# hiboyang/kueue_oss

Hardware: AMD Instinct MI355X
Metric: TAS placements/sec at 128k nodes (1/2/4/8 GPU); % HBM roofline (higher is better)
Workload: dtype int64; 1 GPU; C3: 131072 nodes, 1024 pending workloads per GPU per step from TASPodSetRequests (grouping + request compile + evaluation + TopologyAssignment values in the step; 50% BestFit required/preferred, 50% LeastFreeCapacity unconstrained; taints + nodeSelector); nodes=131072, batch_per_gpu=1024, parallelism=dp1 (replicated snapshot)

## Files before the change

include/kueue_tas.h:

```cpp
#ifndef KUEUE_TAS_H_
#define KUEUE_TAS_H_

#include <stddef.h>
#include <stdint.h>

#ifdef __cplusplus
extern "C" {
#endif

#define KUEUE_TAS_ABI_VERSION 5
#define KUEUE_TAS_MAX_LEVELS 16
#define KUEUE_TAS_MAX_COLS 32
#define KUEUE_TAS_MAX_SELECTORS 8
#define KUEUE_TAS_MAX_LAYERS 4

#define KUEUE_TAS_OK 0
#define KUEUE_TAS_EINVAL -1
#define KUEUE_TAS_ENOMEM -2
#define KUEUE_TAS_EDEVICE -3
#define KUEUE_TAS_ENOSNAPSHOT -4
#define KUEUE_TAS_EOVERFLOW -5
#define KUEUE_TAS_ELAYOUT -6
#define KUEUE_TAS_EHOSTMEM -7

// ... 94 lines not shown
  int32_t excl_affinity;
  int32_t excl_topology;
  int32_t ml_fit[KUEUE_TAS_MAX_LAYERS];
  int32_t ml_need[KUEUE_TAS_MAX_LAYERS];
  int32_t reserved[2];
} kueue_tas_eval_out;

typedef struct {
  int32_t list_cap;
  int32_t max_batch;
  int32_t device;
  int32_t flags;
} kueue_tas_config;
#define KUEUE_TAS_CFG_PACKED_ENTRIES 1
#define KUEUE_TAS_CFG_INLINE_STATS 2
#define KUEUE_TAS_CFG_NO_PAIR_FILL 4
#define KUEUE_TAS_CFG_SERIAL_ADMIT 8
#define KUEUE_TAS_CFG_SPLIT_STATS 16
#define KUEUE_TAS_CFG_FUSED_TOP 32
#define KUEUE_TAS_CFG_HOST_VALUES 64
#define KUEUE_TAS_CFG_NO_CATEGORY_FILL 128
#define KUEUE_TAS_CFG_CLASS_COLLIDE 256
#define KUEUE_TAS_CFG_LFC_IN_FILL 512

int kueue_tas_abi_version(void);
kueue_tas_ctx* kueue_tas_ctx_create(const kueue_tas_config* cfg);
void kueue_tas_ctx_destroy(kueue_tas_ctx* ctx);
const char* kueue_tas_last_error(kueue_tas_ctx* ctx);

int kueue_tas_snapshot_load(kueue_tas_ctx* ctx, const kueue_tas_snapshot_desc* desc);
int kueue_tas_snapshot_apply_deltas(kueue_tas_ctx* ctx, const kueue_tas_delta* deltas, size_t n,
                                    const uint32_t* usage_present_or_null);

int kueue_tas_snapshot_set_free(kueue_tas_ctx* ctx, const int32_t* leaves, size_t n, const int64_t* rows,
                                const uint32_t* free_present);

int kueue_tas_snapshot_set_leaf_attrs(kueue_tas_ctx* ctx, const int32_t* leaves, size_t n, const int32_t* profiles,
                                      const int32_t* labels);

int kueue_tas_snapshot_set_leaf_live(kueue_tas_ctx* ctx, const int32_t* leaves, size_t n, const int32_t* live);

#define KUEUE_TAS_DIGEST_CHUNK 2048
int kueue_tas_snapshot_digest(kueue_tas_ctx* ctx, uint64_t* words, size_t cap, size_t* len, uint64_t* chunks,
                              size_t chunk_cap, size_t* n_chunks);
int kueue_tas_snapshot_read_leaves(kueue_tas_ctx* ctx, const int32_t* leaves, size_t n, int64_t* free_rows,
                                   uint32_t* free_present, int64_t* usage_rows, uint32_t* usage_present,
// ... 170 lines not shown
```

include/kueue_tas_debug.h:

```cpp
#ifndef KUEUE_TAS_DEBUG_H_
#define KUEUE_TAS_DEBUG_H_

#include "kueue_tas.h"

#ifdef __cplusplus
extern "C" {
#endif

int kueue_tas_last_timings(kueue_tas_ctx* ctx, float* ms4);

#define KUEUE_TAS_NUM_STAGES 7
int kueue_tas_last_stage_times(kueue_tas_ctx* ctx, float* ms, int n);

int kueue_tas_last_eval_ticks(kueue_tas_ctx* ctx, int32_t* ticks, size_t n);

int kueue_tas_last_eval_profile(kueue_tas_ctx* ctx, int32_t* ticks, size_t n);
int64_t kueue_tas_last_fill_profile(kueue_tas_ctx* ctx, int32_t* out, size_t n);

int kueue_tas_last_host_times(kueue_tas_ctx* ctx, double* ms, int n);
int kueue_tas_last_host_trace(kueue_tas_ctx* ctx, double* ms, int n);
int64_t kueue_tas_merge_reruns(kueue_tas_ctx* ctx);
int kueue_tas_select_groups(kueue_tas_ctx* ctx, int64_t* last_groups, int64_t* scratch_reruns);
int kueue_tas_last_digest_ms(kueue_tas_ctx* ctx, float* ms2);

int kueue_tas_last_stats(kueue_tas_ctx* ctx, int64_t* stats4);
int64_t kueue_tas_last_alias_fills(kueue_tas_ctx* ctx);
#define KUEUE_TAS_PATH_STAGED 1u
#define KUEUE_TAS_PATH_STAGED_GLOBAL_TAINTS 2u
#define KUEUE_TAS_PATH_GENERIC4 4u
#define KUEUE_TAS_PATH_GENERIC8 8u
#define KUEUE_TAS_PATH_GENERIC16 16u
#define KUEUE_TAS_PATH_GENERIC32 32u
#define KUEUE_TAS_PATH_STAGED_GL 64u
#define KUEUE_TAS_PATH_GLOBAL_STATS 128u
#define KUEUE_TAS_PATH_EXCL 256u
#define KUEUE_TAS_PATH_EXCL_GLOBAL_TAINTS 512u
#define KUEUE_TAS_PATH_SELECTOR_EXT 1024u
#define KUEUE_TAS_PATH_RAGGED_ROLLUP 2048u
#define KUEUE_TAS_PATH_UNIFORM_ROLLUP 4096u
#define KUEUE_TAS_PATH_PAIR 8192u
#define KUEUE_TAS_PATH_ENTRY_TAGS 16384u
#define KUEUE_TAS_PATH_RAGGED_PAIR 32768u
#define KUEUE_TAS_PATH_CATEGORY 65536u
#define KUEUE_TAS_PATH_LFC_FILL 131072u
#define KUEUE_TAS_PATH_FUSED_TOP 262144u
uint32_t kueue_tas_last_fill_paths(kueue_tas_ctx* ctx);
uint64_t kueue_tas_eval_generation(kueue_tas_ctx* ctx);
int kueue_tas_set_stage_timing(kueue_tas_ctx* ctx, int32_t on);
int kueue_tas_snapshot_counters(kueue_tas_ctx* ctx, int64_t* loads, int64_t* splices);
int kueue_tas_device_bytes(kueue_tas_ctx* ctx, int64_t* total, int64_t* phase2);
int kueue_tas_snapshot_usage_mark(kueue_tas_ctx* ctx);
int kueue_tas_snapshot_usage_changes(kueue_tas_ctx* ctx, const kueue_tas_delta** changes, size_t* n);
int kueue_tas_snapshot_apply_deltas_mirrored(kueue_tas_ctx* ctx, const kueue_tas_delta* deltas, size_t n);

int kueue_tas_host_last_timings(kueue_tas_host* h, float* ms4, int64_t* counts3);
int kueue_tas_host_last_stage_times(kueue_tas_host* h, float* ms, int n);
int kueue_tas_host_last_device_host_times(kueue_tas_host* h, double* ms, int n);
int kueue_tas_host_last_eval_profile(kueue_tas_host* h, int32_t* ticks, size_t n);
int kueue_tas_host_last_eval_ticks(kueue_tas_host* h, int32_t* ticks, size_t n);
int kueue_tas_host_last_profile(kueue_tas_host* h, double* ms4);
int kueue_tas_host_last_host_detail(kueue_tas_host* h, double* ms, int n);
int kueue_tas_host_last_update_detail(kueue_tas_host* h, double* ms, int n);
int kueue_tas_host_set_stage_timing(kueue_tas_host* h, int32_t on);
int kueue_tas_host_stage_accum(kueue_tas_host* h, float* ms, int n, int64_t* runs, int64_t* fill_launches,
                               int32_t reset);
int kueue_tas_host_last_stats(kueue_tas_host* h, int64_t* stats8);
int kueue_tas_host_last_stats_ext(kueue_tas_host* h, int64_t* out, int32_t n);
int kueue_tas_host_last_counters(kueue_tas_host* h, size_t workload, int32_t* out, size_t cap);
// ... 13 lines not shown
```

kueue_oss_amd/abi.py:

```python
import ctypes as c

MAX_LEVELS = 16
MAX_COLS = 32
MAX_SELECTORS = 8
MAX_LAYERS = 4

F_REQUIRED = 1
F_UNCONSTRAINED = 2
F_LFC = 4
F_SIMULATE_EMPTY = 8
F_LEADER = 16
F_MULTILAYER = 32
F_AFFINITY = 64
F_DOMAIN = 128
F_SELECTOR_EXT = 256

ST_OK = 0
ST_NO_DOMAINS = 1
ST_NOT_FIT = 2
ST_MULTILAYER = 3
ST_INTERNAL = 4


class SnapshotDesc(c.Structure):
    _fields_ = [
        ("num_levels", c.c_int32),
        ("level_sizes", c.POINTER(c.c_int32)),
        ("child_offsets", c.POINTER(c.c_int32)),
        ("num_cols", c.c_int32),
        ("free_capacity", c.POINTER(c.c_int64)),
        ("tas_usage", c.POINTER(c.c_int64)),
        ("free_present", c.POINTER(c.c_uint32)),
        ("usage_present", c.POINTER(c.c_uint32)),
        ("lowest_is_hostname", c.c_int32),
        ("taint_profile", c.POINTER(c.c_int32)),
        ("num_label_cols", c.c_int32),
        ("label_values", c.POINTER(c.c_int32)),
        ("domain_id_rank", c.POINTER(c.c_int32)),
# ... 183 lines not shown
```

kueue_oss_amd/csrc/tas_device.hip:

```cpp
#include <hip/hip_runtime.h>

#include <algorithm>
#include <chrono>
#include <cstdio>
#include <cstring>
#include <string>
#include <mutex>
#include <unordered_map>
#include <vector>

#include "tas_internal.h"
#include "tas_pool.h"
#include "tas_kernels.hip"

using namespace ktas;

namespace {

constexpr int kEvalsPerFillBlock = kEvalsPerBlock;

bool simple_class(const DevEval& ev, int L) {
  bool simple = (ev.flags & KUEUE_TAS_F_LEADER) == 0 && ev.slice_level == L - 1 && ev.slice_size == 1;
  for (int l = 0; l < L && simple; l++) simple = ev.ssal[l] == 0 || ev.ssal[l] == 1;
  return simple;
// ... 149 lines not shown
  MagicSlot slot[256];
};
void compute_magic(uint64_t d, DevTerm* t, MagicCache& cache) {
  MagicSlot& c = cache.slot[(d * 0x9e3779b97f4a7c15ull) >> 56];
  if (c.d != d) {
    compute_magic_uncached(d, t);
    c.d = d;
    c.magic = t->magic;
    c.shift = t->shift;
    c.add = t->add;
    c.pow2 = t->pow2;
    return;
  }
  t->magic = c.magic;
  t->shift = c.shift;
  t->add = c.add;
  t->pow2 = c.pow2;
}

struct Knobs {
  int admit_grid_sweeps = 6;
  int admit_step_run = 2 * kAdmitWindow;
  int64_t phase2_budget = int64_t(4096) << 20;
  bool force_scratch_rerun = false;
  int64_t lcap_test_cap = 0;
  bool scratch_bounded = true;
  bool lfc_in_fill = false;
  bool emit_after_bf = false;
  int32_t exp_flags = 0;

  static Knobs from_env() {
    Knobs k;
    auto on = [](const char* name) {
      const char* e = getenv(name);
      return e && atoi(e) != 0;
    };
    if (const char* e = getenv("KTAS_ADMIT_PHASES")) k.admit_grid_sweeps = std::max(1, atoi(e));
    if (const char* e = getenv("KTAS_ADMIT_STEP_RUN")) k.admit_step_run = std::max(0, atoi(e));
    if (const char* e = getenv("KTAS_PHASE2_BUDGET")) k.phase2_budget = std::max<int64_t>(atoll(e), 1);
    k.force_scratch_rerun = getenv("KTAS_SCRATCH_TEST_RERUN") != nullptr;
    if (const char* e = getenv("KTAS_SCRATCH_TEST_CAP")) k.lcap_test_cap = std::max<int64_t>(atoll(e), 1);
    k.scratch_bounded = !on("KTAS_SCRATCH_FULL");
    k.lfc_in_fill = on("KTAS_LFC_IN_FILL");
    k.emit_after_bf = on("KTAS_EMIT_MAIN");
    if (const char* e = getenv("KTAS_EXP_FLAGS")) k.exp_flags = int32_t(atoi(e));
    return k;
  }
};

}

struct kueue_tas_ctx {
  int device = 0;
  hipStream_t stream = nullptr;
  hipStream_t stream2 = nullptr;
  hipStream_t stream3 = nullptr;
  hipEvent_t evs[2] = {};
  DevBuf<int8_t> d_fill_lim;
  std::vector<int32_t> cls_pos, cls_cur;
  hipEvent_t ev[8] = {};
  hipEvent_t evl[4] = {};
  std::string err;
  int list_cap = 1024;
  bool inline_stats = true;
  bool pair_fill = true;
  bool admit_window = true;
  Knobs knobs;
  bool fused_top = false;
  bool cat_fill = true;
  bool labels16 = false;
  int64_t n_loads = 0, n_splices = 0;
  bool stage_timing = true;
  int max_batch = 1024;
  int entry_cap = 512;
  bool loaded = false;
  DevSnap snap{};
  int maxD = 0;
  int rack_fanout = 0;
  std::vector<int32_t> h_level_sizes;
  DevBuf<int32_t> d_child_off, d_id_rank, d_taint_profile, d_labels;
  DevBuf<uint8_t> d_dead;
  std::vector<uint8_t> h_dead;
  int64_t n_dead = 0;
  DevBuf<int64_t> d_free, d_usage;
  DevBuf<uint32_t> d_free_present, d_usage_present;
  DevBuf<int32_t> d_counters;
  DevBuf<uint8_t> d_res;
  HostBuf<uint8_t> h_res;
  HostBuf<kueue_tas_eval_out> h_res2;
  kueue_tas_eval_out* res_out_h = nullptr;
  int32_t* res_stats_h = nullptr;
  DevBuf<uint64_t> d_scratch;
  DevBuf<kueue_tas_delta> d_deltas;
  DevBuf<uint8_t> d_setfree;
  DevBuf<uint8_t> d_fits;
  DevBuf<int32_t> d_parent;
  DevBuf<int2> d_wave_tab;
  DevBuf<int32_t> d_leaf_parent;
  DevBuf<char> d_names;
  DevBuf<int64_t> d_name_off;
  bool names_loaded = false;
  DevBuf<char> d_enc_bytes;
  DevBuf<int64_t> d_enc_stroff, d_enc_off;
  DevBuf<int32_t> d_enc_ids, d_enc_counts, d_enc_same;
  DevBuf<kueue_tas_level_enc> d_enc_out;
  DevBuf<int32_t> d_packed;
  DevBuf<LeafPartial> d_partials;
  DevBuf<int32_t> d_fill_stats;
  HostBuf<uint8_t> h_stage;
  DevBuf<uint8_t> d_stage;
  std::vector<int32_t> cls_rep, cls_sig, cls_of, sig_rep, cls_next, sig_next, cls_fastrep, cls_slot, cls_order;
  std::vector<int32_t> sig_base, base_rep, cls_packed, sig_ncls;
// ... 116 lines not shown
  } while (0)

extern "C" {

static double wall_ms() {
  return std::chrono::duration<double, std::milli>(std::chrono::steady_clock::now().time_since_epoch()).count();
}

int kueue_tas_abi_version(void) { return KUEUE_TAS_ABI_VERSION; }

kueue_tas_ctx* kueue_tas_ctx_create(const kueue_tas_config* cfg) {
  DevBufLink* chain = nullptr;
  g_devbuf_chain = &chain;
  auto* c = new kueue_tas_ctx();
  g_devbuf_chain = nullptr;
  c->dev_bufs = chain;
  c->knobs = Knobs::from_env();
  if (cfg) {
    c->device = cfg->device;
    c->inline_stats = (cfg->flags & KUEUE_TAS_CFG_INLINE_STATS) != 0 || (cfg->flags & KUEUE_TAS_CFG_SPLIT_STATS) == 0;
    c->pair_fill = (cfg->flags & KUEUE_TAS_CFG_NO_PAIR_FILL) == 0;
    c->admit_window = (cfg->flags & KUEUE_TAS_CFG_SERIAL_ADMIT) == 0;
    c->fused_top = (cfg->flags & KUEUE_TAS_CFG_FUSED_TOP) != 0;
    c->cat_fill = (cfg->flags & KUEUE_TAS_CFG_NO_CATEGORY_FILL) == 0;
    c->collide_test = (cfg->flags & KUEUE_TAS_CFG_CLASS_COLLIDE) != 0;
    if (cfg->flags & KUEUE_TAS_CFG_LFC_IN_FILL) c->knobs.lfc_in_fill = true;
    if (cfg->list_cap > 0) {
      int lc = 64;
      while (lc < cfg->list_cap && lc < 1024) lc <<= 1;
      c->list_cap = lc;
    }
    if (cfg->max_batch > 0) c->max_batch = cfg->max_batch;
  }
  int ndev = 0;
  if (hipGetDeviceCount(&ndev) != hipSuccess || ndev <= c->device) {
    c->err = "no HIP device available";
    delete c;
    return nullptr;
  }
  int prio_lo = 0, prio_hi = 0;
  if (hipSetDevice(c->device) != hipSuccess || hipDeviceGetStreamPriorityRange(&prio_lo, &prio_hi) != hipSuccess ||
      hipStreamCreateWithPriority(&c->stream, hipStreamNonBlocking, prio_hi) != hipSuccess ||
      hipStreamCreateWithPriority(&c->stream2, hipStreamNonBlocking, prio_hi) != hipSuccess ||
      hipStreamCreateWithPriority(&c->stream3, hipStreamNonBlocking, prio_lo) != hipSuccess) {
    delete c;
    return nullptr;
// ... 45 lines not shown
  c->d_enc_counts.release();
  c->d_enc_same.release();
  c->d_enc_out.release();
  c->d_packed.release();
  c->d_partials.release();
  c->d_fill_stats.release();
  c->h_stage.release();
  c->d_stage.release();
  c->d_overlay.release();
  c->d_rack_pos.release();
  c->d_tags.release();
  c->d_lfc_ch.release();
  c->d_lfc_cp.release();
  c->d_lfc_tot.release();
  c->d_lfc_ovs.release();
  c->d_lfc_ovtot.release();
  c->d_lfc_u8.release();
  c->d_lfc_jobs.release();
  c->d_lfc_items.release();
  c->d_prof.release();
  c->d_level_max.release();
  if (c->ent_host) (void)hipHostFree(c->ent_host);
  c->ent_host = c->ent_dev = nullptr;
  if (c->tag_host) (void)hipHostFree(c->tag_host);
  c->tag_host = c->tag_dev = nullptr;
  c->d_leaf_tags.release();
  for (auto& e : c->ev)
    if (e) (void)hipEventDestroy(e);
  for (auto& e : c->evl)
    if (e) (void)hipEventDestroy(e);
  for (auto& e : c->evs)
    if (e) (void)hipEventDestroy(e);
  if (c->ev_deltas) (void)hipEventDestroy(c->ev_deltas);
  for (auto& e : c->ev_digest)
    if (e) (void)hipEventDestroy(e);
  if (c->stream3) (void)hipStreamDestroy(c->stream3);
  if (c->stream2) (void)hipStreamDestroy(c->stream2);
  if (c->stream) (void)hipStreamDestroy(c->stream);
  delete c;
}

const char* kueue_tas_last_error(kueue_tas_ctx* c) { return c ? c->err.c_str() : "null ctx"; }

static int load_impl(kueue_tas_ctx* c, const kueue_tas_snapshot_desc* d, const kueue_tas_splice_desc* sp);

int kueue_tas_snapshot_load(kueue_tas_ctx* c, const kueue_tas_snapshot_desc* d) { return load_impl(c, d, nullptr); }
// ... 2239 lines not shown
      g_ov += ovf * SD;
      g_tag++;
      max_scr = std::max(max_scr, g_scr);
      max_ov = std::max(max_ov, g_ov);
      max_tag = std::max(max_tag, g_tag);
    }
    groups.push_back(nbf);
    HIPCHK(c, c->d_scratch.ensure(size_t(max_scr)));
    HIPCHK(c, c->d_overlay.ensure(size_t(max_ov)));
    const int ngroups = int(groups.size()) - 1;
    if (c->d_tags.n < size_t(max_tag) * size_t(SD) || c->tag_epoch + ngroups >= 0x7ffffff0) {
      HIPCHK(c, c->d_tags.ensure(size_t(max_tag) * size_t(SD)));
      HIPCHK(c, hipMemsetAsync(c->d_tags.p, 0, c->d_tags.n * 4, c->stream));
      c->tag_epoch = 0;
    }
  }
  c->tag_epoch++;
  const size_t nt = size_t(std::max(a.num_taints, 0));
  p.stats_len = n * nt + n * size_t(s.R) + 3 * n;
  p.res_off_stats = (n * sizeof(kueue_tas_eval_out) + 15) / 16 * 16;
  p.res_bytes = p.res_off_stats + p.stats_len * 4;
  HIPCHK(c, c->d_res.ensure(p.res_bytes));
  HIPCHK(c, c->h_res.ensure(p.res_bytes));
  HIPCHK(c, c->h_res2.ensure(n));
  c->res_out_h = reinterpret_cast<kueue_tas_eval_out*>(c->h_res.p);
  c->res_stats_h = reinterpret_cast<int32_t*>(c->h_res.p + p.res_off_stats);
  p.umask = 0;
  for (size_t i = 0; i < n; i++) p.umask |= hev[i].req_mask | hev[i].lead_mask;
  p.ucols = __builtin_popcount(p.umask);
  p.nstat_all = kStatFixed + int(nt) + s.R;
  p.lds_stats = s.N > 0 && p.nfchunks > 0 && p.ucols <= 8 && p.nstat_all <= kMaxFillStats;
  HIPCHK(c, c->d_lfc_jobs.ensure(n));
  HIPCHK(c, c->d_lfc_items.ensure(size_t(std::max(p.nfast, 1)) * size_t(std::max(nchunks, 1)) + 1));
  const size_t lfc_need = size_t(std::max(nslots * nchunks, 1));
  if (lfc_need > c->lfc_half) {
    c->lfc_half = lfc_need + lfc_need / 4;
    HIPCHK(c, c->d_lfc_ch.ensure(2 * c->lfc_half * kLfcBins));
    HIPCHK(c, c->d_lfc_ovs.ensure(2 * c->lfc_half));
    c->lfc_dirty[0] = c->lfc_dirty[1] = true;
  }
  p.lfc_cur = c->lfc_parity;
  HIPCHK(c, c->d_lfc_cp.ensure(size_t(std::max(nslots * nchunks, 1)) * kLfcBins));
  HIPCHK(c, c->d_lfc_tot.ensure(size_t(std::max(nslots, 1)) * kLfcBins));
  HIPCHK(c, c->d_lfc_ovtot.ensure(size_t(std::max(nslots, 1))));
  HIPCHK(c, c->d_lfc_u8.ensure(size_t(std::max(nslots, 1)) * size_t(std::max(nchunks, 1)) * kLfcChunk));
  p.nblk = (s.N + 255) / 256 * 4;
  HIPCHK(c, c->d_partials.ensure(size_t(std::max(p.nleafsel, 1)) * size_t(std::max(p.nblk, 1))));
  if (c->fused_top) {
// ... 165 lines not shown
  b.aff_vals = reinterpret_cast<const int32_t*>(ds + o.affv);
  b.n = int32_t(n);
  b.num_taints = int32_t(nt);
  b.num_profiles = c->num_profiles;
  b.nstat = 0;
  b.nstat_R = s.R;
  b.fill_stats = nullptr;
  b.stats_split = 0;
  b.fill_lim = nullptr;
  b.cls_member_off = nullptr;
  b.cls_members = nullptr;
  b.rack_fanout = 0;
  b.rack_pos = nullptr;
  b.ctr_sd = s.SD;
  b.counters = c->d_counters.p;
  b.overlay = c->d_overlay.p;
  b.tags = c->d_tags.p;
  b.tag_epoch = c->tag_epoch;
  b.taint_counts = d_stats;
  b.res_counts = d_stats + n * nt;
  b.sel_counts = d_stats + n * nt + n * size_t(s.R);
  b.aff_counts = b.sel_counts + n;
  b.dom_counts = b.aff_counts + n;
  b.out = d_out;
  b.entries = c->ent_dev + c->ent_used;
  b.entry_cap = c->entry_cap;
  b.sel_slots = reinterpret_cast<const SelSlot*>(ds + o.sel);
  b.slot_base = 0;
  b.scratch = c->d_scratch.p;
  b.list_cap = c->list_cap;
  b.nblk = p.nblk;
  b.partials = c->d_partials.p;
  b.partial_idx = reinterpret_cast<const int32_t*>(ds + o.pidx);
  b.rep_of = reinterpret_cast<const int32_t*>(ds + o.rep);
  b.lfc_slot = reinterpret_cast<const int32_t*>(ds + o.slot);
  b.lfc_rep = reinterpret_cast<const int32_t*>(ds + o.lrep);
  b.lfc_nslots = p.nslots;
  b.lfc_nchunks = p.nchunks;
  b.lfc_ch = c->d_lfc_ch.p + size_t(p.lfc_cur) * c->lfc_half * kLfcBins;
  b.lfc_u8 = c->d_lfc_u8.p;
  b.exp_flags = c->knobs.exp_flags;
  b.lfc_cp = c->d_lfc_cp.p;
  b.lfc_tot = c->d_lfc_tot.p;
  b.lfc_ovs = c->d_lfc_ovs.p + size_t(p.lfc_cur) * c->lfc_half;
  b.lfc_ovtot = c->d_lfc_ovtot.p;
  b.lfc_jobs = c->d_lfc_jobs.p;
  b.lfc_nitems = reinterpret_cast<int32_t*>(c->d_lfc_items.p);
// ... 210 lines not shown
  }
  return KUEUE_TAS_OK;
}

static int enqueue_rollup(kueue_tas_ctx* c, const ChunkArgs& a, const ChunkPlan& p, DevBatch& b) {
  const DevSnap& s = c->snap;
  const size_t n = a.n;
  const int nfill = p.nfill, nbf = p.nbf;
  uint8_t* ds = c->d_stage.p;
  const int upper = s.L - 2 - (b.rack_fanout ? 1 : 0);
  int top_parents = 0;
  for (int l = 0; l < upper; l++) top_parents += s.level_size[l];
  const bool fused_top = c->fused_top && nfill > 0 && upper >= 0 && s.level_size[upper] > 0 && top_parents <= 4096 &&
                         s.level_size[upper + 1] / s.level_size[upper] >= 8;
  if (fused_top) {
    c->fill_paths |= KUEUE_TAS_PATH_FUSED_TOP;
    b.level_max = nbf > 0 ? reinterpret_cast<int32_t*>(ds + p.o.top) : nullptr;
    const int per_block = 4 * kParentsPerWave;
    dim3 grid((s.level_size[upper] + per_block - 1) / per_block, unsigned(nfill));
    hipLaunchKernelGGL(rollup_top_kernel, grid, dim3(256), 0, c->stream, s, b, upper,
                       reinterpret_cast<int32_t*>(ds + p.o.top) + n * kMaxLevels);
    HIPCHK(c, hipGetLastError());
  }
  int tail_top = -1;
  if (!fused_top && nfill > 0)
    for (int l = upper; l >= 0 && tail_top < 0; l--)
      if (s.level_size[l] <= kTailParents) tail_top = l;
  for (int l = fused_top ? -1 : upper; l > tail_top; l--) {
    if (s.level_size[l] <= 0) continue;
    const int fanout = s.level_size[l + 1] / s.level_size[l];
    if (fanout >= 8) {
      const int per_block = 4 * kParentsPerWave;
      dim3 grid((s.level_size[l] + per_block - 1) / per_block, unsigned(nfill));
      hipLaunchKernelGGL(rollup_level_wave_kernel, grid, dim3(256), 0, c->stream, s, b, l);
    } else {
      dim3 grid((s.level_size[l] + 255) / 256, unsigned(nfill));
      hipLaunchKernelGGL(rollup_level_kernel, grid, dim3(256), 0, c->stream, s, b, l);
    }
    HIPCHK(c, hipGetLastError());
  }
  if (!fused_top && nfill > 0 && s.L >= 2 && (nbf > 0 || tail_top >= 0)) {
    b.level_max = nullptr;
    if (nbf > 0) {
      HIPCHK(c, c->d_level_max.ensure(size_t(nfill) * size_t(kMaxLevels)));
      b.level_max = c->d_level_max.p;
    }
// ... 67 lines not shown
    HIPCHK(c, hipStreamWaitEvent(c->stream2, c->ev[2], 0));
    if (c->stage_timing) HIPCHK(c, hipEventRecord(c->evl[0], c->stream2));
    if (!b.lfc_fill) {
      hipLaunchKernelGGL(lfc_hist_kernel, dim3(unsigned(nchunks), unsigned(nslots)), dim3(256), 0, c->stream2, s, b);
      HIPCHK(c, hipGetLastError());
    }
    hipLaunchKernelGGL(lfc_total_kernel, dim3(unsigned(nslots)), dim3(kLfcBins), 0, c->stream2, b);
    HIPCHK(c, hipGetLastError());
    if (stats_replicated(p, b)) HIPCHK(c, hipStreamWaitEvent(c->stream2, c->ev[4], 0));
    b.wave_lds = lfc_wave_lds(c);
    const SelSlot* sel = b.sel_slots;
    b.sel_slots = nullptr;
    hipLaunchKernelGGL(select_kernel, dim3(unsigned((nfast + waves - 1) / waves)), dim3(64 * waves),
                       size_t(waves) * size_t(b.wave_lds), c->stream2, s, b, dev_ints(c, p.o.fast), nfast);
    b.sel_slots = sel;
    HIPCHK(c, hipGetLastError());
    if (emit_main) {
      HIPCHK(c, hipEventRecord(c->evl[3], c->stream2));
    } else {
      hipLaunchKernelGGL(lfc_emit_kernel, dim3(unsigned(emit_grid)), dim3(256), 0, c->stream2, s, b);
      HIPCHK(c, hipGetLastError());
    }
    HIPCHK(c, hipEventRecord(c->evl[1], c->stream2));
    HIPCHK(c, hipMemcpyAsync(c->h_res2.p, c->d_res.p, n * sizeof(kueue_tas_eval_out), hipMemcpyDeviceToHost, c->stream2));
  }
  if (nfast && emit_main) {
    HIPCHK(c, hipStreamWaitEvent(c->stream, c->evl[3], 0));
    hipLaunchKernelGGL(lfc_emit_kernel, dim3(unsigned(emit_grid)), dim3(256), 0, c->stream, s, b);
    HIPCHK(c, hipGetLastError());
  }
  return KUEUE_TAS_OK;
}

static int enqueue_results_d2h(kueue_tas_ctx* c, const ChunkPlan& p, const DevBatch& b) {
  if (b.nstat > 0) HIPCHK(c, hipStreamWaitEvent(c->stream, c->evs[1], 0));
  if (c->stage_timing) HIPCHK(c, hipEventRecord(c->ev[7], c->stream));
  HIPCHK(c, hipMemcpyAsync(c->h_res.p, c->d_res.p, p.res_bytes, hipMemcpyDeviceToHost, c->stream));
  return KUEUE_TAS_OK;
}

static bool verify_merge(kueue_tas_ctx* c, const ChunkArgs& a, const ChunkPlan& p) {
  if (c->exact_merge) return true;
  const DevEval* hev = stage_evals(c, p);
  const ClassKeys keys(c, a, p);
  const std::vector<int32_t>& cls_rep = c->cls_rep;
  bool merge_ok = true;
  for (size_t t = 0; t < c->part_cls.size() && merge_ok; t++) {
    const PartClasses& pc = c->part_cls[t];
    for (size_t j = 0; j < pc.rep.size() && merge_ok; j++) {
      const int32_t r = cls_rep[size_t(c->part_map[c->part_base[t] + j])];
      if (r != pc.rep[j]) merge_ok = keys.same_sig(hev[pc.rep[j]], hev[r]) && keys.same_mask(hev[pc.rep[j]], hev[r]);
    }
  }
  for (size_t k = 0; k < cls_rep.size() && merge_ok; k++) {
    const int32_t g = c->sig_rep[size_t(c->cls_sig[k])];
    if (g != cls_rep[k]) merge_ok = keys.same_sig(hev[cls_rep[k]], hev[g]);
  }
  return merge_ok;
}

static int sync_and_check(kueue_tas_ctx* c, const ChunkPlan& p, bool merge_ok) {
  HIPCHK(c, hipStreamSynchronize(c->stream));
  if (p.nfast) {
    HIPCHK(c, hipStreamSynchronize(c->stream2));
    const int32_t* hf = stage_ints(c, p.o.fast);
    for (int k = 0; k < p.nfast; k++) c->res_out_h[hf[k]] = c->h_res2.p[hf[k]];
  }
  if (!merge_ok) {
    c->exact_merge = true;
    c->merge_reruns++;
    return ChunkRerun;
  }
  if (!c->scratch_full && c->knobs.scratch_bounded) {
    const int32_t* hb = stage_ints(c, p.o.bf);
    const SelSlot* hq = reinterpret_cast<const SelSlot*>(c->h_stage.p + p.o.sel);
    for (int k = 0; k < p.nbf; k++) {
      const kueue_tas_eval_out& o = c->res_out_h[hb[k]];
      if ((o.status == KUEUE_TAS_ST_INTERNAL && o.num_workers + o.num_leaders <= c->entry_cap && hq[k].lcap < p.full_lcap) ||
          c->knobs.force_scratch_rerun) {
        c->scratch_full = true;
        c->scratch_reruns++;
        return ChunkRerun;
      }
    }
  }
  return KUEUE_TAS_OK;
}

static int claim_entry_regions(kueue_tas_ctx* c, const ChunkArgs& a) {
  const size_t n = a.n;
// ... 464 lines not shown
```

kueue_oss_amd/csrc/tas_kernels.hip:

```cpp
#include <hip/hip_runtime.h>
#include <stdint.h>

#include <type_traits>

#include "tas_internal.h"

namespace ktas {

__device__ __forceinline__ int32_t w_add(int32_t a, int32_t b) { return int32_t(uint32_t(a) + uint32_t(b)); }
__device__ __forceinline__ int32_t w_sub(int32_t a, int32_t b) { return int32_t(uint32_t(a) - uint32_t(b)); }
__device__ __forceinline__ int32_t w_mul(int32_t a, int32_t b) { return int32_t(uint32_t(a) * uint32_t(b)); }
__device__ __forceinline__ int lane_id();
template <int M>
__device__ __forceinline__ uint32_t bfly(uint32_t v) {
  if constexpr (M == 1) return uint32_t(__builtin_amdgcn_update_dpp(0, int(v), 0xB1, 0xF, 0xF, false));
  else if constexpr (M == 2) return uint32_t(__builtin_amdgcn_update_dpp(0, int(v), 0x4E, 0xF, 0xF, false));
  else if constexpr (M == 4) return uint32_t(__builtin_amdgcn_update_dpp(0, int(v), 0x141, 0xF, 0xF, false));
  else if constexpr (M == 8) return uint32_t(__builtin_amdgcn_update_dpp(0, int(v), 0x140, 0xF, 0xF, false));
  else if constexpr (M == 16) {
    const auto r = __builtin_amdgcn_permlane16_swap(v, v, false, false);
    return uint32_t(r[0]) == v ? uint32_t(r[1]) : uint32_t(r[0]);
  } else {
    static_assert(M == 32, "butterfly steps are 1..32");
    const auto r = __builtin_amdgcn_permlane32_swap(v, v, false, false);
// ... 2169 lines not shown
    int4 v[U];
#pragma unroll
    for (int u = 0; u < U; u++) v[u] = ss4[min(q0 + u * 256 + int(threadIdx.x), nq - 1)];
#pragma unroll
    for (int u = 0; u < U; u++) {
      const int q = q0 + u * 256 + int(threadIdx.x);
      if (q < nq) {
        const int32_t e[4] = {v[u].x, v[u].y, v[u].z, v[u].w};
#pragma unroll
        for (int k = 0; k < 4; k++)
          if (4 * q + k < D) m = max(m, e[k]);
      }
    }
  }
  m = group_reduce(m, 64, OpMax());
  if (lane_id() == 0) red[threadIdx.x >> 6] = m;
  __syncthreads();
  if (threadIdx.x == 0) b.level_max[int64_t(row) * kMaxLevels + l] = max(max(red[0], red[1]), max(red[2], red[3]));
}

__device__ __forceinline__ int32_t load_l2_i32(const int32_t* p) {
  return __hip_atomic_load(p, __ATOMIC_RELAXED, __HIP_MEMORY_SCOPE_AGENT);
}
template <bool L2>
__device__ __forceinline__ void rollup_parent_wave(const DevSnap& s, int32_t* base, int64_t SSO, const DevEval& ev,
                                                   bool leaderReq, int level, int p, int32_t* cmax) {
  const int cl = level + 1;
  const int32_t inner = ev.ssal[cl];
  const bool hasInner = inner != 0;
  const int64_t SD = s.SD;
  const int coff = s.level_off[cl];
  const int lane = lane_id();
  const int cb = s.child_off[s.child_base[level] + p];
  const int ce = s.child_off[s.child_base[level] + p + 1];
  auto ld = [&](int64_t o) { return L2 ? load_l2_i32(base + o) : base[o]; };
  int32_t cap = 0, slc = 0, minD = 0x7fffffff, minSD = 0x7fffffff, lead = 0, mx = INT32_MIN;
  int has = 0;
  for (int c = cb + lane; c < ce; c += kWave) {
    const int g = coff + c;
    int32_t cs = ld(g);
    const int32_t css = ld(SSO + g);
    int32_t csw = cs, csswl = css, cls = 0;
    if (leaderReq) {
      csw = ld(2 * SD + g);
      csswl = ld(3 * SD + g);
      cls = ld(4 * SD + g);
    }
    mx = max(mx, css);
    if (hasInner) {
      cs = w_mul(go_div32(cs, inner), inner);
      csw = w_mul(go_div32(csw, inner), inner);
    }
    cap = w_add(cap, cs);
    slc = w_add(slc, css);
    if (!leaderReq || cls > 0) {
      has = 1;
      minD = min(w_sub(cs, csw), minD);
      minSD = min(w_sub(css, csswl), minSD);
    }
    lead = max(cls, lead);
  }
#pragma unroll
  for (int m = 1; m <= 32; m <<= 1) {
    cap = w_add(cap, xor_lane(cap, m));
    slc = w_add(slc, xor_lane(slc, m));
    minD = min(minD, xor_lane(minD, m));
    minSD = min(minSD, xor_lane(minSD, m));
    lead = max(lead, xor_lane(lead, m));
    has |= xor_lane(has, m);
    mx = max(mx, xor_lane(mx, m));
  }
  *cmax = max(*cmax, mx);
  if (lane == 0) {
    const int32_t state = cap;
    const int32_t swl = has ? w_sub(cap, minD) : 0;
    int32_t sswl = has ? w_sub(slc, minSD) : 0;
    if (level == ev.slice_level) {
      slc = go_div32(state, ev.slice_size);
      sswl = go_div32(swl, ev.slice_size);
    }
    const int g = s.level_off[level] + p;
    base[g] = state;
    if (SSO) base[SD + g] = slc;
    if (leaderReq) {
      base[2 * SD + g] = swl;
      base[3 * SD + g] = sswl;
      base[4 * SD + g] = lead;
    }
  }
}

__global__ __launch_bounds__(256) void rollup_top_kernel(DevSnap s, DevBatch b, int level, int32_t* arrivals) {
  __shared__ int32_t red[4];
  __shared__ int32_t last;
  const int row = blockIdx.y;
  const int eid = b.fill_ids[row];
  const DevEval& ev = b.evals[eid];
  const bool leaderReq = (ev.flags & KUEUE_TAS_F_LEADER) != 0;
  int32_t* base = ctr_base(b, row);
  const int64_t SSO = ss_off(b, row, s.SD);
  const int wv = threadIdx.x >> 6;
  int32_t cmax = INT32_MIN;
  const int p0 = (blockIdx.x * 4 + wv) * kParentsPerWave;
  for (int j = 0; j < kParentsPerWave; j++) {
    const int p = p0 + j;
    if (p < s.level_size[level]) rollup_parent_wave<false>(s, base, SSO, ev, leaderReq, level, p, &cmax);
  }
  if (lane_id() == 0) red[wv] = cmax;
  __syncthreads();
  if (threadIdx.x == 0) {
    const int32_t m = max(max(red[0], red[1]), max(red[2], red[3]));
    if (level + 1 < s.L - 1 && b.level_max) atomicMax(&b.level_max[int64_t(row) * kMaxLevels + level + 1], m);
// ... 41 lines not shown
    const int32_t* ss = base + SSO + s.level_off[l];
    int32_t m = INT32_MIN;
    if (l <= top) {
      for (int i = threadIdx.x; i < s.level_size[l]; i += 256) m = max(m, load_l2_i32(ss + i));
    } else {
      const int D = s.level_size[l];
      const int nq = (D + 3) / 4;
      const int4* ss4 = reinterpret_cast<const int4*>(ss);
      constexpr int U = 4;
      for (int q0 = 0; q0 < nq; q0 += U * 256) {
        int4 v[U];
#pragma unroll
        for (int u = 0; u < U; u++) v[u] = ss4[min(q0 + u * 256 + int(threadIdx.x), nq - 1)];
#pragma unroll
        for (int u = 0; u < U; u++) {
          const int q = q0 + u * 256 + int(threadIdx.x);
          const int32_t e[4] = {v[u].x, v[u].y, v[u].z, v[u].w};
#pragma unroll
          for (int k = 0; k < 4; k++)
            if (q < nq && 4 * q + k < D) m = max(m, e[k]);
        }
      }
    }
    m = group_reduce(m, 64, OpMax());
    if (lane_id() == 0) red[wv] = m;
    __syncthreads();
    if (threadIdx.x == 0) b.level_max[int64_t(row) * kMaxLevels + l] = max(max(red[0], red[1]), max(red[2], red[3]));
    __syncthreads();
  }
}

__global__ __launch_bounds__(kFillThreads) void leaf_partials_kernel(DevSnap s, DevBatch b, const int32_t* ids,
                                                                    int nids) {
  const int e0 = blockIdx.y * kEvalsPerBlock;
  const int ne = min(kEvalsPerBlock, nids - e0);
  const int leaf = blockIdx.x * kFillThreads + threadIdx.x;
  const bool valid = leaf < s.N;
  const int gleaf = s.level_off[s.L - 1] + leaf;
  const int lane = lane_id();
  const int64_t SD = s.SD;
  for (int e = 0; e < ne; e++) {
    const int eid = uni(ids[e0 + e]);
    const DevEval& ev = b.evals[eid];
    const uint32_t flags = uint32_t(uni(int32_t(ev.flags)));
    const bool leader = (flags & KUEUE_TAS_F_LEADER) != 0;
    const bool lfc = (flags & KUEUE_TAS_F_LFC) != 0;
// ... 4067 lines not shown
```

kueue_oss_amd/native.py:

```python
from __future__ import annotations

import ctypes
import json
import os
import subprocess

_PKG = os.path.dirname(os.path.abspath(__file__))
_CSRC = os.path.join(_PKG, "csrc")
_BUILD = os.path.join(_PKG, "_build")
_LIB = None


class NativeLibraryMissing(RuntimeError):
    """libkueue_tas.so could not be loaded or no HIP device is usable."""


def library_path() -> str:
    return os.path.join(_BUILD, "libkueue_tas.so")


def build_native(jobs: int = 4) -> str:
    subprocess.run(["make", "-s", f"-j{jobs}", "-C", _CSRC], check=True)
    return library_path()

# ... 207 lines not shown


def resource_quantity_string(name: str, value: int, lib=None) -> str:
    lib = lib if lib is not None else load_library()
    buf = ctypes.create_string_buffer(64)
    n = ctypes.c_size_t()
    if lib.kueue_tas_resource_quantity_string(name.encode(), value, buf, 64, ctypes.byref(n)):
        raise RuntimeError("kueue_tas_resource_quantity_string failed")
    return buf.value.decode()


def _take(lib, p) -> dict:
    s = ctypes.cast(p, ctypes.c_char_p).value.decode()
    lib.kueue_tas_free(p)
    return json.loads(s)


class TASFlavorSnapshot:

    def __init__(self, snapshot: dict, list_cap: int = 0, max_batch: int = 0, device: int = 0, lib=None,
                 packed_entries: bool = False, inline_stats: bool = False,
                 pair_fill: bool = True, serial_admit: bool = False, split_stats: bool = False,
                 fused_top: bool = False, host_values: bool = False, category_fill: bool = True,
                 class_collide: bool = False, lfc_in_fill: bool = False):
        self._lib = lib if lib is not None else load_library()
        cfg = KueueTasConfig(list_cap, max_batch, device, (1 if packed_entries else 0) | (2 if inline_stats else 0)
                              | (0 if pair_fill else 4) | (8 if serial_admit else 0) | (16 if split_stats else 0)
                              | (32 if fused_top else 0) | (64 if host_values else 0)
                              | (0 if category_fill else 128) | (256 if class_collide else 0)
                              | (512 if lfc_in_fill else 0))
        doc = {k: v for k, v in snapshot.items() if k != "podSets"}
        h = self._lib.kueue_tas_host_create(json.dumps(doc).encode(), ctypes.byref(cfg))
        if not h:
            raise NativeLibraryMissing("kueue_tas_host_create returned NULL")
        err = self._lib.kueue_tas_host_last_error(h).decode()
        if err:
            self._lib.kueue_tas_host_destroy(h)
            raise NativeLibraryMissing(err)
        self._h = h

    def close(self):
        if getattr(self, "_h", None):
            self._lib.kueue_tas_host_destroy(self._h)
            self._h = None

    def __del__(self):
        try:
            self.close()
        except Exception:
            pass

    def _err(self):
        return self._lib.kueue_tas_host_last_error(self._h).decode()
# ... 452 lines not shown
```

Baseline: 3.692 million placements/s.

## Write eval results to mapped host memory; add optional LDS block rollup kernel

```diff
diff --git a/include/kueue_tas.h b/include/kueue_tas.h
--- a/include/kueue_tas.h
+++ b/include/kueue_tas.h
@@ -140,6 +140,8 @@
 #define KUEUE_TAS_CFG_NO_CATEGORY_FILL 128
 #define KUEUE_TAS_CFG_CLASS_COLLIDE 256
 #define KUEUE_TAS_CFG_LFC_IN_FILL 512
+#define KUEUE_TAS_CFG_BLOCK_ROLLUP 1024
+#define KUEUE_TAS_CFG_COPY_RESULTS 2048
 
 int kueue_tas_abi_version(void);
 kueue_tas_ctx* kueue_tas_ctx_create(const kueue_tas_config* cfg);
diff --git a/include/kueue_tas_debug.h b/include/kueue_tas_debug.h
--- a/include/kueue_tas_debug.h
+++ b/include/kueue_tas_debug.h
@@ -44,6 +44,7 @@
 #define KUEUE_TAS_PATH_CATEGORY 65536u
 #define KUEUE_TAS_PATH_LFC_FILL 131072u
 #define KUEUE_TAS_PATH_FUSED_TOP 262144u
+#define KUEUE_TAS_PATH_BLOCK_ROLLUP 524288u
 uint32_t kueue_tas_last_fill_paths(kueue_tas_ctx* ctx);
 uint64_t kueue_tas_eval_generation(kueue_tas_ctx* ctx);
 int kueue_tas_set_stage_timing(kueue_tas_ctx* ctx, int32_t on);
diff --git a/kueue_oss_amd/abi.py b/kueue_oss_amd/abi.py
--- a/kueue_oss_amd/abi.py
+++ b/kueue_oss_amd/abi.py
@@ -14,6 +14,11 @@
 F_AFFINITY = 64
 F_DOMAIN = 128
 F_SELECTOR_EXT = 256
+
+CFG_BLOCK_ROLLUP = 1024
+CFG_COPY_RESULTS = 2048
+
+PATH_BLOCK_ROLLUP = 1 << 19
 
 ST_OK = 0
 ST_NO_DOMAINS = 1
diff --git a/kueue_oss_amd/csrc/tas_device.hip b/kueue_oss_amd/csrc/tas_device.hip
--- a/kueue_oss_amd/csrc/tas_device.hip
+++ b/kueue_oss_amd/csrc/tas_device.hip
@@ -195,6 +195,8 @@
   int admit_grid_sweeps = 6;
   int admit_step_run = 2 * kAdmitWindow;
   int64_t phase2_budget = int64_t(4096) << 20;
+  bool block_rollup = false;
+  int64_t rollup_lds_budget = 12288;
   bool force_scratch_rerun = false;
   int64_t lcap_test_cap = 0;
   bool scratch_bounded = true;
@@ -211,11 +213,13 @@
     if (const char* e = getenv("KTAS_ADMIT_PHASES")) k.admit_grid_sweeps = std::max(1, atoi(e));
     if (const char* e = getenv("KTAS_ADMIT_STEP_RUN")) k.admit_step_run = std::max(0, atoi(e));
     if (const char* e = getenv("KTAS_PHASE2_BUDGET")) k.phase2_budget = std::max<int64_t>(atoll(e), 1);
+    if (const char* e = getenv("KTAS_ROLLUP_LDS_BUDGET")) k.rollup_lds_budget = std::max<int64_t>(atoll(e), 0);
     k.force_scratch_rerun = getenv("KTAS_SCRATCH_TEST_RERUN") != nullptr;
     if (const char* e = getenv("KTAS_SCRATCH_TEST_CAP")) k.lcap_test_cap = std::max<int64_t>(atoll(e), 1);
     k.scratch_bounded = !on("KTAS_SCRATCH_FULL");
     k.lfc_in_fill = on("KTAS_LFC_IN_FILL");
     k.emit_after_bf = on("KTAS_EMIT_MAIN");
+    k.block_rollup = on("KTAS_BLOCK_ROLLUP");
     if (const char* e = getenv("KTAS_EXP_FLAGS")) k.exp_flags = int32_t(atoi(e));
     return k;
   }
@@ -240,6 +244,7 @@
   bool admit_window = true;
   Knobs knobs;
   bool fused_top = false;
+  bool mapped_results = true;
   bool cat_fill = true;
   bool labels16 = false;
   int64_t n_loads = 0, n_splices = 0;
@@ -261,6 +266,9 @@
   DevBuf<uint8_t> d_res;
   HostBuf<uint8_t> h_res;
   HostBuf<kueue_tas_eval_out> h_res2;
+  kueue_tas_eval_out* res_map_host = nullptr;
+  kueue_tas_eval_out* res_map_dev = nullptr;
+  size_t res_map_cap = 0;
   kueue_tas_eval_out* res_out_h = nullptr;
   int32_t* res_stats_h = nullptr;
   DevBuf<uint64_t> d_scratch;
@@ -423,6 +431,8 @@
     c->pair_fill = (cfg->flags & KUEUE_TAS_CFG_NO_PAIR_FILL) == 0;
     c->admit_window = (cfg->flags & KUEUE_TAS_CFG_SERIAL_ADMIT) == 0;
     c->fused_top = (cfg->flags & KUEUE_TAS_CFG_FUSED_TOP) != 0;
+    if (cfg->flags & KUEUE_TAS_CFG_BLOCK_ROLLUP) c->knobs.block_rollup = true;
+    c->mapped_results = (cfg->flags & KUEUE_TAS_CFG_COPY_RESULTS) == 0;
     c->cat_fill = (cfg->flags & KUEUE_TAS_CFG_NO_CATEGORY_FILL) == 0;
     c->collide_test = (cfg->flags & KUEUE_TAS_CFG_CLASS_COLLIDE) != 0;
     if (cfg->flags & KUEUE_TAS_CFG_LFC_IN_FILL) c->knobs.lfc_in_fill = true;
@@ -514,6 +524,8 @@
   c->d_level_max.release();
   if (c->ent_host) (void)hipHostFree(c->ent_host);
   c->ent_host = c->ent_dev = nullptr;
+  if (c->res_map_host) (void)hipHostFree(c->res_map_host);
+  c->res_map_host = c->res_map_dev = nullptr;
   if (c->tag_host) (void)hipHostFree(c->tag_host);
   c->tag_host = c->tag_dev = nullptr;
   c->d_leaf_tags.release();
@@ -2799,8 +2811,21 @@
   p.res_bytes = p.res_off_stats + p.stats_len * 4;
   HIPCHK(c, c->d_res.ensure(p.res_bytes));
   HIPCHK(c, c->h_res.ensure(p.res_bytes));
-  HIPCHK(c, c->h_res2.ensure(n));
-  c->res_out_h = reinterpret_cast<kueue_tas_eval_out*>(c->h_res.p);
+  if (c->mapped_results) {
+    if (n > c->res_map_cap) {
+      const size_t cap = std::max<size_t>(n, 2 * c->res_map_cap);
+      kueue_tas_eval_out* q = nullptr;
+      HIPCHK(c, hipHostMalloc(&q, cap * sizeof(kueue_tas_eval_out), hipHostMallocMapped | hipHostMallocCoherent));
+      if (c->res_map_host) (void)hipHostFree(c->res_map_host);
+      c->res_map_host = q;
+      c->res_map_cap = cap;
+      HIPCHK(c, hipHostGetDevicePointer(reinterpret_cast<void**>(&c->res_map_dev), q, 0));
+    }
+    c->res_out_h = c->res_map_host;
+  } else {
+    HIPCHK(c, c->h_res2.ensure(n));
+    c->res_out_h = reinterpret_cast<kueue_tas_eval_out*>(c->h_res.p);
+  }
   c->res_stats_h = reinterpret_cast<int32_t*>(c->h_res.p + p.res_off_stats);
   p.umask = 0;
   for (size_t i = 0; i < n; i++) p.umask |= hev[i].req_mask | hev[i].lead_mask;
@@ -3012,7 +3037,7 @@
   b.sel_counts = d_stats + n * nt + n * size_t(s.R);
   b.aff_counts = b.sel_counts + n;
   b.dom_counts = b.aff_counts + n;
-  b.out = d_out;
+  b.out = c->mapped_results ? c->res_map_dev : d_out;
   b.entries = c->ent_dev + c->ent_used;
   b.entry_cap = c->entry_cap;
   b.sel_slots = reinterpret_cast<const SelSlot*>(ds + o.sel);
@@ -3269,6 +3294,25 @@
                        reinterpret_cast<int32_t*>(ds + p.o.top) + n * kMaxLevels);
     HIPCHK(c, hipGetLastError());
   }
+  if (c->knobs.block_rollup && !fused_top && nfill > 0 && upper >= 0 && s.level_size[upper + 1] > 0) {
+    int64_t fields = 1;
+    for (int k = 0; k < nfill; k++) fields = std::max<int64_t>(fields, c->ctr_row_off[size_t(k) + 1] - c->ctr_row_off[size_t(k)]);
+    const int64_t mirror = fields * s.level_off[upper + 2];
+    if (fields * s.level_size[upper + 1] <= c->knobs.rollup_lds_budget && mirror <= kBlockRollupLarge) {
+      c->fill_paths |= KUEUE_TAS_PATH_BLOCK_ROLLUP;
+      b.level_max = nullptr;
+      if (nbf > 0) {
+        HIPCHK(c, c->d_level_max.ensure(size_t(nfill) * size_t(kMaxLevels)));
+        b.level_max = c->d_level_max.p;
+      }
+      if (mirror <= kBlockRollupSmall)
+        hipLaunchKernelGGL(rollup_block_kernel<kBlockRollupSmall>, dim3(unsigned(nfill)), dim3(256), 0, c->stream, s, b, upper);
+      else
+        hipLaunchKernelGGL(rollup_block_kernel<kBlockRollupLarge>, dim3(unsigned(nfill)), dim3(256), 0, c->stream, s, b, upper);
+      HIPCHK(c, hipGetLastError());
+      return KUEUE_TAS_OK;
+    }
+  }
   int tail_top = -1;
   if (!fused_top && nfill > 0)
     for (int l = upper; l >= 0 && tail_top < 0; l--)
@@ -3382,7 +3426,8 @@
       HIPCHK(c, hipGetLastError());
     }
     HIPCHK(c, hipEventRecord(c->evl[1], c->stream2));
-    HIPCHK(c, hipMemcpyAsync(c->h_res2.p, c->d_res.p, n * sizeof(kueue_tas_eval_out), hipMemcpyDeviceToHost, c->stream2));
+    if (!c->mapped_results)
+      HIPCHK(c, hipMemcpyAsync(c->h_res2.p, c->d_res.p, n * sizeof(kueue_tas_eval_out), hipMemcpyDeviceToHost, c->stream2));
   }
   if (nfast && emit_main) {
     HIPCHK(c, hipStreamWaitEvent(c->stream, c->evl[3], 0));
@@ -3393,6 +3438,14 @@
 }
 
 static int enqueue_results_d2h(kueue_tas_ctx* c, const ChunkPlan& p, const DevBatch& b) {
+  if (c->mapped_results) {
+    if (c->stage_timing) HIPCHK(c, hipEventRecord(c->ev[7], c->stream));
+    if (b.nstat == 0) HIPCHK(c, hipStreamWaitEvent(c->stream3, stats_replicated(p, b) ? c->ev[4] : c->ev[2], 0));
+    if (p.stats_len)
+      HIPCHK(c, hipMemcpyAsync(c->h_res.p + p.res_off_stats, c->d_res.p + p.res_off_stats, p.stats_len * 4,
+                               hipMemcpyDeviceToHost, c->stream3));
+    return KUEUE_TAS_OK;
+  }
   if (b.nstat > 0) HIPCHK(c, hipStreamWaitEvent(c->stream, c->evs[1], 0));
   if (c->stage_timing) HIPCHK(c, hipEventRecord(c->ev[7], c->stream));
   HIPCHK(c, hipMemcpyAsync(c->h_res.p, c->d_res.p, p.res_bytes, hipMemcpyDeviceToHost, c->stream));
@@ -3423,9 +3476,12 @@
   HIPCHK(c, hipStreamSynchronize(c->stream));
   if (p.nfast) {
     HIPCHK(c, hipStreamSynchronize(c->stream2));
-    const int32_t* hf = stage_ints(c, p.o.fast);
-    for (int k = 0; k < p.nfast; k++) c->res_out_h[hf[k]] = c->h_res2.p[hf[k]];
-  }
+    if (!c->mapped_results) {
+      const int32_t* hf = stage_ints(c, p.o.fast);
+      for (int k = 0; k < p.nfast; k++) c->res_out_h[hf[k]] = c->h_res2.p[hf[k]];
+    }
+  }
+  if (c->mapped_results) HIPCHK(c, hipStreamSynchronize(c->stream3));
   if (!merge_ok) {
     c->exact_merge = true;
     c->merge_reruns++;
diff --git a/kueue_oss_amd/csrc/tas_kernels.hip b/kueue_oss_amd/csrc/tas_kernels.hip
--- a/kueue_oss_amd/csrc/tas_kernels.hip
+++ b/kueue_oss_amd/csrc/tas_kernels.hip
@@ -2215,29 +2215,37 @@
 __device__ __forceinline__ int32_t load_l2_i32(const int32_t* p) {
   return __hip_atomic_load(p, __ATOMIC_RELAXED, __HIP_MEMORY_SCOPE_AGENT);
 }
-template <bool L2>
-__device__ __forceinline__ void rollup_parent_wave(const DevSnap& s, int32_t* base, int64_t SSO, const DevEval& ev,
-                                                   bool leaderReq, int level, int p, int32_t* cmax) {
+#if defined(__HIP_DEVICE_COMPILE__)
+typedef __attribute__((address_space(3))) int32_t lds_i32;
+#else
+typedef int32_t lds_i32;
+#endif
+template <bool L2, bool MIR = false>
+__device__ __forceinline__ void rollup_parent_range(const DevSnap& s, int32_t* base, int64_t SSO, bool leaderReq, int level,
+                                                    int32_t inner, bool at_slice, int32_t slice_size, int p, int cb, int ce,
+                                                    int32_t* cmax, lds_i32* mirror = nullptr, int MSD = 0) {
   const int cl = level + 1;
-  const int32_t inner = ev.ssal[cl];
   const bool hasInner = inner != 0;
   const int64_t SD = s.SD;
   const int coff = s.level_off[cl];
   const int lane = lane_id();
-  const int cb = s.child_off[s.child_base[level] + p];
-  const int ce = s.child_off[s.child_base[level] + p + 1];
-  auto ld = [&](int64_t o) { return L2 ? load_l2_i32(base + o) : base[o]; };
+  const int MSS = SSO ? MSD : 0;
+  auto ld = [&](int f, int g) {
+    if (MIR) return int32_t(mirror[(f == 1 ? MSS : f * MSD) + g]);
+    const int64_t o = (f == 1 ? SSO : f * SD) + g;
+    return L2 ? load_l2_i32(base + o) : base[o];
+  };
   int32_t cap = 0, slc = 0, minD = 0x7fffffff, minSD = 0x7fffffff, lead = 0, mx = INT32_MIN;
   int has = 0;
   for (int c = cb + lane; c < ce; c += kWave) {
     const int g = coff + c;
-    int32_t cs = ld(g);
-    const int32_t css = ld(SSO + g);
+    int32_t cs = ld(0, g);
+    const int32_t css = ld(1, g);
     int32_t csw = cs, csswl = css, cls = 0;
     if (leaderReq) {
-      csw = ld(2 * SD + g);
-      csswl = ld(3 * SD + g);
-      cls = ld(4 * SD + g);
+      csw = ld(2, g);
+      csswl = ld(3, g);
+      cls = ld(4, g);
     }
     mx = max(mx, css);
     if (hasInner) {
@@ -2268,9 +2276,9 @@
     const int32_t state = cap;
     const int32_t swl = has ? w_sub(cap, minD) : 0;
     int32_t sswl = has ? w_sub(slc, minSD) : 0;
-    if (level == ev.slice_level) {
-      slc = go_div32(state, ev.slice_size);
-      sswl = go_div32(swl, ev.slice_size);
+    if (at_slice) {
+      slc = go_div32(state, slice_size);
+      sswl = go_div32(swl, slice_size);
     }
     const int g = s.level_off[level] + p;
     base[g] = state;
@@ -2280,7 +2288,24 @@
       base[3 * SD + g] = sswl;
       base[4 * SD + g] = lead;
     }
-  }
+    if (MIR) {
+      mirror[g] = state;
+      if (SSO) mirror[MSD + g] = slc;
+      if (leaderReq) {
+        mirror[2 * MSD + g] = swl;
+        mirror[3 * MSD + g] = sswl;
+        mirror[4 * MSD + g] = lead;
+      }
+    }
+  }
+}
+template <bool L2>
+__device__ __forceinline__ void rollup_parent_wave(const DevSnap& s, int32_t* base, int64_t SSO, const DevEval& ev,
+                                                   bool leaderReq, int level, int p, int32_t* cmax) {
+  const int cb = s.child_off[s.child_base[level] + p];
+  const int ce = s.child_off[s.child_base[level] + p + 1];
+  rollup_parent_range<L2>(s, base, SSO, leaderReq, level, ev.ssal[level + 1], level == ev.slice_level, ev.slice_size, p, cb,
+                          ce, cmax);
 }
 
 __global__ __launch_bounds__(256) void rollup_top_kernel(DevSnap s, DevBatch b, int level, int32_t* arrivals) {
@@ -2368,6 +2393,72 @@
         }
       }
     }
+    m = group_reduce(m, 64, OpMax());
+    if (lane_id() == 0) red[wv] = m;
+    __syncthreads();
+    if (threadIdx.x == 0) b.level_max[int64_t(row) * kMaxLevels + l] = max(max(red[0], red[1]), max(red[2], red[3]));
+    __syncthreads();
+  }
+}
+
+constexpr int kBlockRollupSmall = 5120;
+constexpr int kBlockRollupLarge = 15360;
+template <int CAP>
+__global__ __launch_bounds__(256) void rollup_block_kernel(DevSnap s, DevBatch b, int upper) {
+  __shared__ int32_t mirror[CAP];
+  __shared__ int32_t red[4];
+  const int row = blockIdx.x;
+  const DevEval& ev = b.evals[b.fill_ids[row]];
+  const bool leaderReq = (ev.flags & KUEUE_TAS_F_LEADER) != 0;
+  int32_t* base = ctr_base(b, row);
+  const int64_t SD = s.SD;
+  const int64_t SSO = ss_off(b, row, SD);
+  const int nf = leaderReq ? 5 : SSO ? 2 : 1;
+  const int cl = upper + 1;
+  const int MSD = s.level_off[cl + 1];
+  const int wv = threadIdx.x >> 6;
+  {
+    const int coff = s.level_off[cl];
+    const int nq = (s.level_size[cl] + 3) / 4;
+    const int total = nf * nq;
+    constexpr int U = 4;
+    for (int q0 = 0; q0 < total; q0 += U * 256) {
+      int4 v[U];
+#pragma unroll
+      for (int u = 0; u < U; u++) {
+        const int i = min(q0 + u * 256 + int(threadIdx.x), total - 1);
+        const int f = i / nq;
+        v[u] = reinterpret_cast<const int4*>(base + f * SD + coff)[i - f * nq];
+      }
+#pragma unroll
+      for (int u = 0; u < U; u++) {
+        const int i = min(q0 + u * 256 + int(threadIdx.x), total - 1);
+        const int f = i / nq;
+        reinterpret_cast<int4*>(mirror + f * MSD + coff)[i - f * nq] = v[u];
+      }
+    }
+  }
+  __syncthreads();
+  for (int l = upper; l >= 0; l--) {
+    const int np = s.level_size[l];
+    const int32_t* coffs = s.child_off + s.child_base[l];
+    const int32_t inner = ev.ssal[l + 1], slice_size = ev.slice_size;
+    const bool at_slice = l == ev.slice_level;
+    int32_t unused = INT32_MIN;
+    for (int p0 = wv; p0 < np; p0 += 4 * kWave) {
+      const int mine = min(p0 + 4 * lane_id(), np - 1);
+      const int cbs = coffs[mine], ces = coffs[mine + 1];
+      for (int j = 0; j < kWave && p0 + 4 * j < np; j++)
+        rollup_parent_range<false, true>(s, base, SSO, leaderReq, l, inner, at_slice, slice_size, p0 + 4 * j, bcast(cbs, j),
+                                         bcast(ces, j), &unused, (lds_i32*)mirror, MSD);
+    }
+    __syncthreads();
+  }
+  if (!b.level_max) return;
+  for (int l = 0; l <= cl && l + 1 < s.L; l++) {
+    const int32_t* ss = mirror + (SSO ? MSD : 0) + s.level_off[l];
+    int32_t m = INT32_MIN;
+    for (int i = threadIdx.x; i < s.level_size[l]; i += 256) m = max(m, ss[i]);
     m = group_reduce(m, 64, OpMax());
     if (lane_id() == 0) red[wv] = m;
     __syncthreads();
diff --git a/kueue_oss_amd/native.py b/kueue_oss_amd/native.py
--- a/kueue_oss_amd/native.py
+++ b/kueue_oss_amd/native.py
@@ -253,13 +253,15 @@
                  packed_entries: bool = False, inline_stats: bool = False,
                  pair_fill: bool = True, serial_admit: bool = False, split_stats: bool = False,
                  fused_top: bool = False, host_values: bool = False, category_fill: bool = True,
-                 class_collide: bool = False, lfc_in_fill: bool = False):
+                 class_collide: bool = False, lfc_in_fill: bool = False, block_rollup: bool = False,
+                 copy_results: bool = False):
         self._lib = lib if lib is not None else load_library()
         cfg = KueueTasConfig(list_cap, max_batch, device, (1 if packed_entries else 0) | (2 if inline_stats else 0)
                               | (0 if pair_fill else 4) | (8 if serial_admit else 0) | (16 if split_stats else 0)
                               | (32 if fused_top else 0) | (64 if host_values else 0)
                               | (0 if category_fill else 128) | (256 if class_collide else 0)
-                              | (512 if lfc_in_fill else 0))
+                              | (512 if lfc_in_fill else 0) | (1024 if block_rollup else 0)
+                              | (2048 if copy_results else 0))
         doc = {k: v for k, v in snapshot.items() if k != "podSets"}
         h = self._lib.kueue_tas_host_create(json.dumps(doc).encode(), ctypes.byref(cfg))
         if not h:
```

Result: slower. 3.535 million placements/s (-4.3%).
